# alinjar1996/manipulator_mujoco

Measured on AMD Instinct MI355X. Metric: candidate rollouts/sec (N×H steps) UR5e scene, 1/2/4/8 MI355X, higher is better.
Workload: dtype f32; 1 GPU; C3 scene_mjx: UR5e+Hand-E arm + object.xml box (URD/scene_mjx.xml), Newton(1 it, 5 ls), 4096 candidates x 50 steps per GPU, order-10 Bernstein, dt 0.05; candidates_per_gpu=4096, horizon=50, global_batch=4096, parallelism=dp1 (candidate shards; key exchange), world_size_seen=1, backend=single process, gpus_visible=1, launcher=single process, exchange=none (one rank: the fused atomic-min key is the global best)

## Files before the change

manipulator_mujoco_amd/build.py:

```python

from __future__ import annotations

import os
import shutil
import subprocess
import sys

HERE = os.path.dirname(os.path.abspath(__file__))
CSRC = os.path.join(HERE, "csrc")
_ROLLOUT_FLAGS = ["-Xarch_device", "-fno-slp-vectorize", "-Xarch_device", "-fassociative-math",
                  "-Xarch_device", "-fno-signed-zeros", "-Xarch_device", "-fno-trapping-math"]
UNITS = [(os.path.join(CSRC, "engine.hip"), [], False),
         (os.path.join(CSRC, "rollout_narrow.hip"), _ROLLOUT_FLAGS, False),
         (os.path.join(CSRC, "rollout_wide.hip"), _ROLLOUT_FLAGS, True)]
SRC = [u[0] for u in UNITS]
DEPS = SRC + [os.path.join(CSRC, f) for f in ("rollout.hip", "rollout.h", "cem.hip", "comm.hip",
                                              "mpcr_device.h", "mjcf_embed.cpp")] + [
    os.path.join(os.path.dirname(HERE), "include", f) for f in ("mpcr.h", "mpcr_model.h", "mpcr_mjcf.h")]
OUT = os.path.join(HERE, "libmpcr.so")
ARCH = os.environ.get("MPCR_OFFLOAD_ARCH", "gfx950")
FLAGS = ["-O3", "-std=c++17", "-fPIC", "-Wall", "-Wno-pass-failed",
         "-fno-hip-fp32-correctly-rounded-divide-sqrt", "-Xarch_device", "-freciprocal-math",
         "-Xarch_device", "-fapprox-func", "-mllvm", "-simplifycfg-sink-common=false"]


def source_hash() -> str:
    import hashlib
    h = hashlib.sha256()
    for d in DEPS:
        h.update(os.path.basename(d).encode())
        with open(d, "rb") as f:
            h.update(f.read())
    h.update(repr((FLAGS, [u[1:] for u in UNITS])).encode())
    return h.hexdigest()[:16]


def hipcc():
    for c in (os.environ.get("HIPCC"), "/opt/rocm/bin/hipcc", shutil.which("hipcc")):
        if c and os.path.exists(c):
            return c
    raise RuntimeError("hipcc not found")


FAST_MATH = {"-freciprocal-math", "-fapprox-func", "-fassociative-math", "-fno-signed-zeros", "-fno-trapping-math"}


def _drop_fast(flags):
    out, skip = [], False
    for i, f in enumerate(flags):
# ... 65 lines not shown
```

manipulator_mujoco_amd/csrc/engine.hip:

```cpp
#include <hip/hip_runtime.h>
#include <dlfcn.h>

#include <algorithm>
#include <atomic>
#include <cfloat>
#include <cmath>
#include <cstdarg>
#include <cstdio>
#include <cstring>
#include <limits>
#include <string>
#include <thread>
#include <vector>

#include "../../include/mpcr.h"
#include "mpcr_device.h"

#include "rollout.h"

#ifndef MPCR_SEG_STEPS_DEFAULT
#define MPCR_SEG_STEPS_DEFAULT 7
#endif
#ifndef MPCR_SEG_GROUPS_DEFAULT
#define MPCR_SEG_GROUPS_DEFAULT 2
#endif
#define MPCR_SEG_MAXG 4
static int env_int_or(const char* name, int dflt) {
  const char* v = getenv(name);
  return v ? atoi(v) : dflt;
}
#include "cem.hip"

namespace mpcr {
__global__ void __launch_bounds__(256) argmin_kernel(const float* __restrict__ cost, int stride, int n, int base,
                                                     unsigned long long* key) {
  unsigned long long best = ~0ull;
  for (int i = blockIdx.x * blockDim.x + threadIdx.x; i < n; i += gridDim.x * blockDim.x) {
    const float c = cost[(size_t)i * stride];
    const uint32_t u = __float_as_uint(c);
    const uint32_t k = isnan(c) ? 0u : ((u & 0x80000000u) ? ~u : (u | 0x80000000u));
    const unsigned long long k64 = ((unsigned long long)k << 32) | (uint32_t)(base + i);
    best = k64 < best ? k64 : best;
  }
#pragma unroll
  for (int o = 32; o > 0; o >>= 1) {
    const unsigned long long other = __shfl_xor(best, o);
    best = other < best ? other : best;
  }
  if ((threadIdx.x & 63) == 0) atomicMin(key, best);
}

// ... 14 lines not shown
  DevModel* d_model = nullptr;
  float* d_pdot = nullptr;
  float* d_in = nullptr;
  float* d_cost = nullptr;
  float* d_theta = nullptr;
  float* d_thetadot = nullptr;
  unsigned long long* d_key = nullptr;
  int* d_status = nullptr;
  int* d_idx = nullptr;
  float* d_slot_prev = nullptr;
  float* d_jx = nullptr;
  float* d_td = nullptr;
  short* d_hints = nullptr;
  unsigned* d_pace = nullptr;
  float* d_mslab = nullptr;
  float* d_seg = nullptr;
  int seg_steps = 0, seg_groups = 1, seg_min_n = 0;
  hipStream_t seg_stream[MPCR_SEG_MAXG] = {};
  hipEvent_t seg_event[MPCR_SEG_MAXG + 1] = {};
  float4* d_hull_vert = nullptr;
  int2* d_hull_info = nullptr;
  float4* d_hull_adjv = nullptr;
  float4* d_hull_head = nullptr;
  float4* d_hull_lut = nullptr;
  float4* d_face_plane = nullptr;
  int2* d_face_vinfo = nullptr;
  int* d_face_vert = nullptr;
  int2* d_vert_finfo = nullptr;
  int* d_vert_face = nullptr;
  int2* d_cone_cell = nullptr;
  int* d_cone_face = nullptr;
  bool wide = false;
};

static bool needs_wide(const mpcr_model_t& m, const DevModel& d) {
  if (m.nv > 16 || d.nbody > 16 || d.ngeom > 24 || m.nq > MPCR_N_NQ || m.nu > 0 || d.has_spring ||
      m.integrator != MPCR_INT_EULER || m.cone != MPCR_CONE_PYRAMIDAL || m.nten > 0 || m.viscosity != 0)
    return true;
  for (int e = 0; e < m.neq; e++)
    if (m.eq_type[e] != MPCR_EQ_JOINT) return true;
  for (int p = 0; p < m.npair; p++)
    if (m.pair_func[p] == MPCR_COL_CONVEX || m.pair_func[p] == MPCR_COL_PLANE_CONVEX) return true;
  return false;
}

static thread_local std::string g_err;

static int fail(int code, const char* fmt, ...) __attribute__((format(printf, 2, 3)));
static int fail(int code, const char* fmt, ...) {
  char buf[512];
  va_list ap;
  va_start(ap, fmt);
  vsnprintf(buf, sizeof(buf), fmt, ap);
  va_end(ap);
  g_err = buf;
  return code;
}

#define HIPCHK(x)                                                                         \
  do {                                                                                    \
    hipError_t e_ = (x);                                                                  \
    if (e_ != hipSuccess) return fail(MPCR_EHIP, "%s: %s", #x, hipGetErrorString(e_));  \
  } while (0)

extern "C" const char* mpcr_last_error(void) { return g_err.c_str(); }
extern "C" int mpcr_abi_version(void) { return MPCR_ABI_VERSION; }
// ... 847 lines not shown
        double ctr[3], cr[3];
        dir(0.5 * (u0 + u1), 0.5 * (v0 + v1), ctr);
        double rad = 0.0;
        for (double u : {u0, u1})
          for (double v : {v0, v1}) {
            dir(u, v, cr);
            const double cd = ctr[0] * cr[0] + ctr[1] * cr[1] + ctr[2] * cr[2];
            rad = std::max(rad, std::acos(std::min(1.0, cd)));
          }
        const double cth = std::cos(thr0 + rad);
        const int start = (int)cface.size();
        for (int f = fa; f < fa + fnum; f++) {
          const double* fp = h.face_plane[f];
          const double fn = std::sqrt(fp[0] * fp[0] + fp[1] * fp[1] + fp[2] * fp[2]);
          if (fn > 0 && (fp[0] * ctr[0] + fp[1] * ctr[1] + fp[2] * ctr[2]) / fn >= cth) cface.push_back(f);
        }
        ccell.push_back(make_int2(start, (int)cface.size() - start));
      }
    }
    if (cface.empty()) cface.push_back(0);
    if (ccell.empty()) ccell.push_back(make_int2(0, 0));
    if (hipMalloc(&e->d_cone_cell, sizeof(int2) * ccell.size()) != hipSuccess ||
        hipMalloc(&e->d_cone_face, sizeof(int) * cface.size()) != hipSuccess ||
        hipMemcpy(e->d_cone_cell, ccell.data(), sizeof(int2) * ccell.size(), hipMemcpyHostToDevice) != hipSuccess ||
        hipMemcpy(e->d_cone_face, cface.data(), sizeof(int) * cface.size(), hipMemcpyHostToDevice) != hipSuccess) {
      mpcr_engine_free(e);
      return fail(MPCR_ENOMEM, "cone table upload failed");
    }
    e->dev.cone_cell = as_gmem(e->d_cone_cell);
    e->dev.cone_face = as_gmem(e->d_cone_face);
  }
  const int nc = e->host.nctrl;
  const size_t in_cols = (size_t)nc * (horizon > nbasis ? horizon : nbasis);
  if (hipMalloc(&e->d_model, sizeof(DevModel)) != hipSuccess ||
      hipMalloc(&e->d_pdot, sizeof(float) * horizon * nbasis) != hipSuccess ||
      hipMalloc(&e->d_in, sizeof(float) * max_n * in_cols) != hipSuccess ||
      hipMalloc(&e->d_cost, sizeof(float) * max_n * 4) != hipSuccess ||
      hipMalloc(&e->d_theta, sizeof(float) * max_n * nc * horizon) != hipSuccess ||
      hipMalloc(&e->d_thetadot, sizeof(float) * max_n * nc * horizon) != hipSuccess ||
      hipMalloc(&e->d_key, sizeof(unsigned long long)) != hipSuccess ||
      hipMalloc(&e->d_status, sizeof(int) * max_n) != hipSuccess ||
      hipMalloc(&e->d_idx, sizeof(int) * max_n) != hipSuccess ||
      hipMalloc(&e->d_slot_prev, sizeof(float) * ((size_t)max_n + 1) * (e->host.nslot > 0 ? e->host.nslot : 1)) !=
          hipSuccess ||
      hipMalloc(&e->d_jx, sizeof(float) * ((size_t)max_n + 1) *
                              (e->wide ? (SmemW::MAXEFC - SmemW::JL + 1) * SmemW::LDJ
                                       : (SmemN::MAXEFC - SmemN::JL + 1) * SmemN::LDJ)) !=
          hipSuccess ||
      hipMalloc(&e->d_hints, sizeof(short) * 2 * (size_t)max_n * (e->wide ? SmemW::NHINT : 1)) != hipSuccess ||
      hipMalloc(&e->d_pace, sizeof(unsigned) * MPCR_PACE_SLOTS) != hipSuccess ||
      hipMalloc(&e->d_mslab, sizeof(float) * ((size_t)max_n + 1) * (e->wide ? SmemW::NVW * SmemW::LD : 1)) !=
          hipSuccess ||
      hipMalloc(&e->d_td, sizeof(float) * ((size_t)max_n + 1) * (size_t)(e->host.nctrl > 0 ? e->host.nctrl : 1) *
                              (size_t)horizon) != hipSuccess) {
    mpcr_engine_free(e);
    return fail(MPCR_ENOMEM, "device allocation failed");
  }
  if (hipMemcpy(e->d_model, &e->dev, sizeof(DevModel), hipMemcpyHostToDevice) != hipSuccess ||
      hipMemcpy(e->d_pdot, pdot, sizeof(float) * horizon * nbasis, hipMemcpyHostToDevice) != hipSuccess ||
      hipMemset(e->d_hints, 0xff, sizeof(short) * 2 * (size_t)max_n * (e->wide ? SmemW::NHINT : 1)) !=
          hipSuccess ||
      hipMemset(e->d_pace, 0xff, sizeof(unsigned) * MPCR_PACE_SLOTS) != hipSuccess) {
    mpcr_engine_free(e);
    return fail(MPCR_EHIP, "model upload failed");
  }
  if (e->wide) {
    e->seg_steps = env_int_or("MPCR_SEG_STEPS", MPCR_SEG_STEPS_DEFAULT);
    e->seg_groups = std::max(1, std::min(MPCR_SEG_MAXG, env_int_or("MPCR_SEG_GROUPS", MPCR_SEG_GROUPS_DEFAULT)));
    if (e->seg_steps > 0 && e->seg_steps < horizon) {
      int occ[6] = {0, 0, 0, 0, 0, 0}, ncu = 0;
      if (rollout_occupancy(occ) == hipSuccess &&
          hipDeviceGetAttribute(&ncu, hipDeviceAttributeMultiprocessorCount, device) == hipSuccess)
        e->seg_min_n = occ[3] * ncu;
      bool ok = hipMalloc(&e->d_seg, sizeof(float) * (size_t)max_n * SEG_STRIDE) == hipSuccess;
      for (int g = 0; ok && e->seg_groups > 1 && g < e->seg_groups; g++)
        ok = hipStreamCreateWithFlags(&e->seg_stream[g], hipStreamNonBlocking) == hipSuccess;
      for (int g = 0; ok && e->seg_groups > 1 && g <= e->seg_groups; g++)
        ok = hipEventCreateWithFlags(&e->seg_event[g], hipEventDisableTiming) == hipSuccess;
      if (!ok) {
        mpcr_engine_free(e);
        return fail(MPCR_ENOMEM, "horizon-segment state allocation failed");
      }
    }
  }
  *out = e;
  return MPCR_OK;
}

extern "C" void mpcr_engine_free(mpcr_engine* e) {
// ... 798 lines not shown
```

manipulator_mujoco_amd/csrc/rollout.hip:

```cpp
#pragma once
#include "rollout.h"
#include "../../include/mpcr_model.h"

namespace mpcr {

#ifdef MPCR_PROFILE
#define PROF_DECL unsigned long long prof_acc[32] = {0}; unsigned long long prof_last = __builtin_amdgcn_s_memtime();
#define STAMP(i)                                              \
  do {                                                        \
    unsigned long long now_ = __builtin_amdgcn_s_memtime();   \
    prof_acc[i] += now_ - prof_last;                          \
    prof_last = now_;                                         \
  } while (0)
#define PROF_FLUSH                                                          \
  if (lane == 0 && args.prof)                                               \
    for (int i_ = 0; i_ < 32; i_++) atomicAdd(&args.prof[i_ + 32 * (threadIdx.x >> 6)], prof_acc[i_]);
#ifdef MPCR_PROFILE_COUNTS
#define PROF_COUNT(m, i)                                                                  \
  do {                                                                                    \
    if ((m)->prof && (int)__lane_id() == __builtin_ctzll(__ballot(1))) atomicAdd((m)->prof + (i), 1ull); \
  } while (0)
#else
#define PROF_COUNT(m, i)
#endif
#define PSTAMP_DECL unsigned long long pst_ = __builtin_amdgcn_s_memtime();
#define PSTAMP(m, i)                                                                       \
  do {                                                                                     \
    const unsigned long long now_ = __builtin_amdgcn_s_memtime();                          \
    if ((m)->prof && (int)__lane_id() == 0) atomicAdd((m)->prof + (i) + 32 * (threadIdx.x >> 6), now_ - pst_); \
    pst_ = now_;                                                                           \
  } while (0)
#else
#define PSTAMP_DECL
#define PSTAMP(m, i)
// ... 8 lines not shown
  if (ahead >= 3) __builtin_amdgcn_s_setprio(3); \
  else if (ahead == 2) __builtin_amdgcn_s_setprio(2); \
  else if (ahead == 1) __builtin_amdgcn_s_setprio(1); \
  else __builtin_amdgcn_s_setprio(0); \
  }

#ifndef MPCR_CB_SKIP
#define MPCR_CB_SKIP 1
#endif
#ifdef MPCR_STOP_AFTER
#define STOP_AT(k) \
  if (MPCR_STOP_AFTER == (k)) continue;
#else
#define STOP_AT(k)
#endif


#if defined(__HIP_DEVICE_COMPILE__)
#define ASSUME_GLOBAL(p) __builtin_assume(!__builtin_amdgcn_is_shared((const void*)(p)) && \
                                          !__builtin_amdgcn_is_private((const void*)(p)))
#define ASSUME_LDS(p) __builtin_assume(__builtin_amdgcn_is_shared((const void*)(p)))
#define ASSUME_PRIVATE(p) __builtin_assume(__builtin_amdgcn_is_private((const void*)(p)))
#else
#define ASSUME_GLOBAL(p)
#define ASSUME_LDS(p)
#define ASSUME_PRIVATE(p)
#endif
__device__ __forceinline__ const MPCR_GMEM DevModel* uniform_model(const DevModel* p) {
  const unsigned long long a = reinterpret_cast<unsigned long long>(p);
  const unsigned lo = __builtin_amdgcn_readfirstlane((unsigned)a), hi = __builtin_amdgcn_readfirstlane((unsigned)(a >> 32));
  return reinterpret_cast<const MPCR_GMEM DevModel*>(((unsigned long long)hi << 32) | lo);
}

__device__ __forceinline__ float rdlane(float v, int l) {
  return __int_as_float(__builtin_amdgcn_readlane(__float_as_int(v), l));
}
template <int CTRL>
__device__ __forceinline__ float dppf(float v) {
  return __int_as_float(__builtin_amdgcn_update_dpp(0, __float_as_int(v), CTRL, 0xF, 0xF, false));
}
template <int CTRL, int ROWS>
__device__ __forceinline__ float dppf_rows(float v) {
  return __int_as_float(__builtin_amdgcn_update_dpp(0, __float_as_int(v), CTRL, ROWS, 0xF, false));
}
__device__ __forceinline__ float wsum(float v) {
  v += dppf<0xB1>(v);
  v += dppf<0x4E>(v);
  v += dppf<0x124>(v);
  v += dppf<0x128>(v);
  v += dppf_rows<0x142, 0xA>(v);
  v += dppf_rows<0x143, 0xC>(v);
  return rdlane(v, 63);
}
__device__ __forceinline__ int lanes_below(unsigned long long mask) {
  return (int)__builtin_amdgcn_mbcnt_hi((unsigned)(mask >> 32), __builtin_amdgcn_mbcnt_lo((unsigned)mask, 0u));
}
template <int BITS = 3>
__device__ __forceinline__ int wscan_excl(int v, int& total) {
  int pre = 0, tot = 0;
#pragma unroll
  for (int bit = 0; bit < BITS; bit++) {
    const unsigned long long mk = __ballot((v >> bit) & 1);
    pre += lanes_below(mk) << bit;
    tot += __popcll(mk) << bit;
  }
  total = tot;
// ... 2339 lines not shown
  float vnext = lane < nc ? tdp[lane * H + t_begin] : 0.f;
  float cost_g = 0.f, cost_r = 0.f, cost_c = 0.f;
  SlotHist<S> shist;
#pragma unroll
  for (int j = 0; j < SlotHist<S>::NC; j++)
#pragma unroll
    for (int c = 0; c < 4; c++) shist.v[j][c] = 0.f;
  int status = 0, nefc_sum = 0, nefc_max = 0;
  if (resume) {
    cost_c = segs[SEG_COSTC + lane];
    const float* sc = segs + SEG_SCAL;
    cost_g = sc[0]; cost_r = sc[1];
    status = __float_as_int(sc[2]); nefc_sum = __float_as_int(sc[3]); nefc_max = __float_as_int(sc[4]);
  }
  const int ctrl_qa = lane < nc ? m->ctrl_qposadr[lane] : 0, ctrl_da = lane < nc ? m->ctrl_dofadr[lane] : 0;
  PROF_DECL
  unsigned* pace = nullptr;
  int pace_own = 0;
  unsigned pace_v = ~0u;
  if (WPC == 1 && args.pace) {
    const unsigned hw = __builtin_amdgcn_s_getreg((31 << 11) | 4);
    const unsigned xcc = __builtin_amdgcn_s_getreg((3 << 11) | 20);
    const unsigned grp = ((((xcc & 7u) * 8u + ((hw >> 13) & 7u)) * 2u + ((hw >> 12) & 1u)) * 16u + ((hw >> 8) & 15u)) *
                             4u + ((hw >> 4) & 3u);
    pace = args.pace + grp * 16u;
    pace_own = (int)(hw & 15u);
  }
#ifdef MPCR_WAVETIME
  const unsigned long long wt_t0 = __builtin_amdgcn_s_memrealtime(), wt_c0 = __builtin_amdgcn_s_memtime();
  unsigned wt_newton = 0, wt_ls = 0, wt_cvx = 0;
#endif

  auto cdof_phase = [&]() {
    if (lane < nv) {
      const int bd = m->dof_body[lane], kind = m->dof_kind[lane];
      const int tr = m->body_tree[bd];
      float* c = s.cdof[lane];
      float R[9];
#pragma unroll
      for (int k = 0; k < 9; k++) R[k] = s.xmat[bd][k];
      if (kind == 2) {
        c[0] = c[1] = c[2] = 0.f;
        const int k = m->dof_sub[lane];
        c[3] = k == 0 ? 1.f : 0.f;
        c[4] = k == 1 ? 1.f : 0.f;
        c[5] = k == 2 ? 1.f : 0.f;
      } else {
        float ax[3], anchor[3];
        if (kind == 3) {
          const int k = m->dof_sub[lane];
          ax[0] = s.xmat[bd][k]; ax[1] = s.xmat[bd][3 + k]; ax[2] = s.xmat[bd][6 + k];
          anchor[0] = s.xpos[bd][0]; anchor[1] = s.xpos[bd][1]; anchor[2] = s.xpos[bd][2];
        } else {
          const int j = m->dof_jnt[lane];
          float w[3];
          mv(ax, R, m->jnt_axis[j]);
          mv(w, R, m->jnt_pos[j]);
          anchor[0] = s.xpos[bd][0] + w[0]; anchor[1] = s.xpos[bd][1] + w[1]; anchor[2] = s.xpos[bd][2] + w[2];
        }
        if (kind == 1) {
          c[0] = c[1] = c[2] = 0.f;
          c[3] = ax[0]; c[4] = ax[1]; c[5] = ax[2];
        } else {
          float off[3] = {s.com[tr][0] - anchor[0], s.com[tr][1] - anchor[1], s.com[tr][2] - anchor[2]}, cr[3];
          cross(cr, ax, off);
          c[0] = ax[0]; c[1] = ax[1]; c[2] = ax[2];
          c[3] = cr[0]; c[4] = cr[1]; c[5] = cr[2];
        }
      }
    }
  };
  for (int t = t_begin; t < t_end; t++) {
    LAUNDER_MODEL();
    LAUNDER_LANE();
    if (pace) {
      if (lane == pace_own) __hip_atomic_store(pace + lane, (unsigned)t, __ATOMIC_RELAXED, __HIP_MEMORY_SCOPE_WORKGROUP);
      if (lane < 16) pace_v = __hip_atomic_load(pace + lane, __ATOMIC_RELAXED, __HIP_MEMORY_SCOPE_AGENT);
    }
    if (run_main) {
    if (lane < nc) {
      const float v = vnext;
      if (t + 1 < H) vnext = tdp[lane * H + t + 1];
      s.qvel[ctrl_da] = v;
      if (args.layout != 0 && args.thetadot) args.thetadot[(size_t)b * nc * H + lane * H + t] = v;
    }
    sync();

    STAMP(0);
    STOP_AT(0)
    {
      float q[4] = {1.f, 0.f, 0.f, 0.f}, p[3] = {0.f, 0.f, 0.f};
      int anc = -1;
      if (lane < nb) {
        const int kind = m->body_kind[lane];
        const int j = m->body_jnt[lane];
        q[0] = m->body_bquat[lane][0]; q[1] = m->body_bquat[lane][1];
        q[2] = m->body_bquat[lane][2]; q[3] = m->body_bquat[lane][3];
        p[0] = m->body_bpos[lane][0]; p[1] = m->body_bpos[lane][1]; p[2] = m->body_bpos[lane][2];
        anc = m->body_anc[lane];
        if (kind == BK_FREE) {
          const int a = m->jnt_qposadr[j];
          p[0] = s.qpos[a]; p[1] = s.qpos[a + 1]; p[2] = s.qpos[a + 2];
          q[0] = s.qpos[a + 3]; q[1] = s.qpos[a + 4]; q[2] = s.qpos[a + 5]; q[3] = s.qpos[a + 6];
          float n = sqrtf(q[0] * q[0] + q[1] * q[1] + q[2] * q[2] + q[3] * q[3]);
          if (n < kMinVal) { q[0] = 1.f; q[1] = q[2] = q[3] = 0.f; }
          else { q[0] /= n; q[1] /= n; q[2] /= n; q[3] /= n; }
          anc = -1;
        } else if (kind == BK_HINGE || kind == BK_SLIDE) {
          const float qa = s.qpos[m->jnt_qposadr[j]] - m->jnt_qpos0[j];
          const float* ax = m->jnt_axis[j];
          float R[9];
          q2m(R, q);
          if (kind == BK_SLIDE) {
            float w[3];
            mv(w, R, ax);
            p[0] += w[0] * qa; p[1] += w[1] * qa; p[2] += w[2] * qa;
          } else {
            float sn, cs;
            __sincosf(0.5f * qa, &sn, &cs);
            float qj[4] = {cs, ax[0] * sn, ax[1] * sn, ax[2] * sn}, Rj[9], c[3], rc[3], d[3], w[3];
            c[0] = m->jnt_pos[j][0]; c[1] = m->jnt_pos[j][1]; c[2] = m->jnt_pos[j][2];
            q2m(Rj, qj);
            mv(rc, Rj, c);
            d[0] = c[0] - rc[0]; d[1] = c[1] - rc[1]; d[2] = c[2] - rc[2];
            mv(w, R, d);
            p[0] += w[0]; p[1] += w[1]; p[2] += w[2];
            qmul(q, q, qj);
          }
        }
      }
      for (int r = 0; r < m->jump_rounds; r++) {
        const int src = anc >= 0 ? anc : lane;
        float aq[4], ap[3];
        aq[0] = wshfl(q[0], src); aq[1] = wshfl(q[1], src);
        aq[2] = wshfl(q[2], src); aq[3] = wshfl(q[3], src);
        ap[0] = wshfl(p[0], src); ap[1] = wshfl(p[1], src); ap[2] = wshfl(p[2], src);
        const int aanc = wshfl(anc, src);
        if (anc >= 0) {
          float R[9], w[3];
          q2m(R, aq);
          mv(w, R, p);
          p[0] = ap[0] + w[0]; p[1] = ap[1] + w[1]; p[2] = ap[2] + w[2];
          qmul(q, aq, q);
          anc = aanc;
        }
      }
      if (lane < nb) {
        float n = sqrtf(q[0] * q[0] + q[1] * q[1] + q[2] * q[2] + q[3] * q[3]);
        q[0] /= n; q[1] /= n; q[2] /= n; q[3] /= n;
        float R[9], w[3];
        q2m(R, q);
        s.xpos[lane][0] = p[0]; s.xpos[lane][1] = p[1]; s.xpos[lane][2] = p[2];
        s.xquat[lane][0] = q[0]; s.xquat[lane][1] = q[1]; s.xquat[lane][2] = q[2]; s.xquat[lane][3] = q[3];
#pragma unroll
        for (int k = 0; k < 9; k++) s.xmat[lane][k] = R[k];
        mv(w, R, m->body_ipos[lane]);
        s.xipos[lane][0] = p[0] + w[0]; s.xipos[lane][1] = p[1] + w[1]; s.xipos[lane][2] = p[2] + w[2];
      }
    }
    sync();

    STAMP(1);
    STOP_AT(1)
    if (lane < m->ngeom) {
      const int gb = m->geom_body[lane];
      float gq[4] = {m->geom_quat[lane][0], m->geom_quat[lane][1], m->geom_quat[lane][2], m->geom_quat[lane][3]};
      float Rg[9];
      q2m(Rg, gq);
      if (gb < 0) {
        s.gxpos[lane][0] = m->geom_pos[lane][0]; s.gxpos[lane][1] = m->geom_pos[lane][1];
        s.gxpos[lane][2] = m->geom_pos[lane][2];
#pragma unroll
        for (int k = 0; k < 9; k++) s.gxmat[lane][k] = Rg[k];
      } else {
        float w[3], R[9], Rr[9];
#pragma unroll
        for (int k = 0; k < 9; k++) R[k] = s.xmat[gb][k];
        mv(w, R, m->geom_pos[lane]);
        s.gxpos[lane][0] = s.xpos[gb][0] + w[0]; s.gxpos[lane][1] = s.xpos[gb][1] + w[1];
        s.gxpos[lane][2] = s.xpos[gb][2] + w[2];
#pragma unroll
        for (int i = 0; i < 3; i++)
#pragma unroll
          for (int k = 0; k < 3; k++)
            Rr[3 * i + k] = R[3 * i] * Rg[k] + R[3 * i + 1] * Rg[3 + k] + R[3 * i + 2] * Rg[6 + k];
#pragma unroll
        for (int k = 0; k < 9; k++) s.gxmat[lane][k] = Rr[k];
      }
    }
// ... 618 lines not shown
        STAMP(18);
      }
      if (split && !lead && run_coll && lane == 0) s.ncon = ncon_w;
      sync();
      if (run_coll && s.ncon > S::MAXACT) {
        status |= 1;
        sync();
        if (lane == 0) s.ncon = S::MAXACT;
        sync();
      }
    }
    const bool rows_c = WPC == 2 && m->coll_rows;
    const bool rows_j = WPC == 2 && S::WIDE && !rows_c;
    const bool hess2 = rows_j && NVW == 32;
    const bool impl2 = hess2 && S::WIDE && m->integrator == 3 && !m->impl_cross && blk_usable<NVW>(m);
    constexpr int BLK_N = NVW == 16 ? 8 : 16;
    static_assert(!S::SPLIT || (BLK_N + 1) * WAVE <= S::DYN_FLOATS, "the implicit factor inside the dynamics region");
    float* const implf = &s.xpos[0][0];
    const int rl0 = rows_j ? wv * WAVE : 0, rls = rows_j ? 2 * WAVE : WAVE;
    if constexpr (WPC == 2) {
      if (!rows_c) {
        block_sync();
        if (!run_main && !rows_j) continue;
      }
    }

    STAMP(7);
    STOP_AT(7)
    bool coupled = true;
    if (WPC == 1 || rows_j || (rows_c ? run_coll : run_main)) {
      const int ncon = s.ncon;
      const int neq = (m->disableflags & 64) ? 0 : (S::WIDE ? m->neqrow : m->neq);
      int nlim_l = 0, lsides = 0;
      if (lane < m->njnt && !(m->disableflags & 32) && m->jnt_limited[lane] &&
          (m->jnt_type[lane] == 2 || m->jnt_type[lane] == 3)) {
        const float q = s.qpos[m->jnt_qposadr[lane]];
        if (q - m->jnt_range[lane][0] < m->jnt_margin[lane]) { nlim_l++; lsides |= 1; }
        if (m->jnt_range[lane][1] - q < m->jnt_margin[lane]) { nlim_l++; lsides |= 2; }
      }
      int nlim;
      const int lim_pre = wscan_excl(nlim_l, nlim);
      int ntr = 0, tsides = 0;
      if constexpr (S::WIDE) {
        if (!(m->disableflags & 32))
          for (int t = 0; t < m->nten; t++) {
            if (!m->ten_limited[t]) continue;
            const float dx = s.tenp[t][1][0] - s.tenp[t][0][0], dy = s.tenp[t][1][1] - s.tenp[t][0][1],
                        dz = s.tenp[t][1][2] - s.tenp[t][0][2];
            const float len = sqrtf(dx * dx + dy * dy + dz * dz);
            if (len - m->ten_range[t][0] < m->ten_margin[t]) { tsides |= 1 << (2 * t); ntr++; }
            if (m->ten_range[t][1] - len < m->ten_margin[t]) { tsides |= 2 << (2 * t); ntr++; }
          }
      }
      const bool ell = S::WIDE && m->cone == 1;
      int ncr = 0;
      if (lane < ncon) ncr = m->pair_condim[s.con_pair[lane]] == 1 ? 1 : (ell ? 3 : 4);
      int ncrow;
      const int con_pre = wscan_excl(ncr, ncrow);
      int nefc = neq + nlim + ntr + ncrow;
      int keep_con = ncon;
      if (nefc > S::MAXEFC) {
        const int room = S::MAXEFC - neq - nlim - ntr;
        const unsigned long long fit = __ballot(lane < ncon && con_pre + ncr <= room);
        keep_con = __popcll(fit);
        nefc = neq + nlim + ntr + (keep_con > 0 ? wshfl(con_pre + ncr, keep_con - 1) : 0);
        status |= 1;
// ... 103 lines not shown
                            s.con_pos[c][2] - s.com[tr][2]}, cr[3];
              cross(cr, cd, r);
              const float sg = side == 0 ? -1.f : 1.f;
              jd[0] += sg * (cd[3] + cr[0]); jd[1] += sg * (cd[4] + cr[1]); jd[2] += sg * (cd[5] + cr[2]);
            }
          }
        }
        float fw[9];
        const float* f = s.con_frame[c];
        if constexpr (S::FRAMEW == 3) {
          make_frame(fw, s.con_frame[c]);
          f = fw;
        }
        const float jn = f[0] * jd[0] + f[1] * jd[1] + f[2] * jd[2];
        const int off = s.con_row[c];
        if (m->pair_condim[p] == 1) {
          jstore(s, gx, off, i, jn);
        } else if (S::WIDE && m->cone == 1) {
          jstore(s, gx, off + 0, i, jn);
          jstore(s, gx, off + 1, i, f[3] * jd[0] + f[4] * jd[1] + f[5] * jd[2]);
          jstore(s, gx, off + 2, i, f[6] * jd[0] + f[7] * jd[1] + f[8] * jd[2]);
        } else {
          const float mu = m->pair_friction[p];
          const float jt1 = f[3] * jd[0] + f[4] * jd[1] + f[5] * jd[2];
          const float jt2 = f[6] * jd[0] + f[7] * jd[1] + f[8] * jd[2];
          jstore(s, gx, off + 0, i, jn + mu * jt1);
          jstore(s, gx, off + 1, i, jn - mu * jt1);
          jstore(s, gx, off + 2, i, jn + mu * jt2);
          jstore(s, gx, off + 3, i, jn - mu * jt2);
        }
      }
      if (rows_j) block_sync();
      else sync();
      for (int r = lane + rl0; r < nefc; r += rls) {
        const int src = s.efc_src[r], kind = src >> 24, id = (src >> 4) & 0xfffff, side = src & 15;
        float pos, margin, diag;
        const float* sref;
        const float* simp;
        if (S::WIDE && kind == 1 && side > 0) {
          pos = s.eqp[id][0][side - 1] - s.eqp[id][1][side - 1];
          margin = 0.f;
          diag = m->eq_diag[id];
          sref = m->eq_solref[id];
          simp = m->eq_solimp[id];
        } else if (kind == 1) {
          const int j1 = m->eq_j1[id], j2 = m->eq_j2[id];
          const float* c = m->eq_data[id];
          const float q1 = s.qpos[m->jnt_qposadr[j1]] - m->jnt_qpos0[j1];
          if (j2 >= 0) {
            const float dif = s.qpos[m->jnt_qposadr[j2]] - m->jnt_qpos0[j2];
            pos = q1 - (c[0] + dif * (c[1] + dif * (c[2] + dif * (c[3] + dif * c[4]))));
          } else {
            pos = q1 - c[0];
          }
          margin = 0.f;
          diag = m->eq_diag[id];
          sref = m->eq_solref[id];
          simp = m->eq_solimp[id];
        } else if (kind == 2) {
          const float q = s.qpos[m->jnt_qposadr[id]];
          pos = side == 0 ? q - m->jnt_range[id][0] : m->jnt_range[id][1] - q;
          margin = m->jnt_margin[id];
          diag = m->dof_invweight0[m->jnt_dofadr[id]];
          sref = m->jnt_solref[id];
          simp = m->jnt_solimp[id];
        } else if (S::WIDE && kind == 4) {
// ... 538 lines not shown
```

Baseline: 2.555 million rollouts/s.

## Add precomputed per-body/dof/row step table with packed float4 loads for narrow rollout

Builds a host-side step table of per-body kinematics constants, per-dof descriptors and per-constraint-row impedance and solref parameters (K, B, reciprocals, power flags). The table is packed as aligned float4 records and placed behind the device model. The narrow rollout kernel reads it in kinematics, cdof and constraint-row phases instead of scattered DevModel fields and per-step solimp/solref arithmetic. Intent is fewer scalar global loads and less repeated parameter math per step. The cost is extra device memory and a second code path that must stay consistent with the model, which a host-side equivalence check enforces.

```diff
diff --git a/manipulator_mujoco_amd/build.py b/manipulator_mujoco_amd/build.py
--- a/manipulator_mujoco_amd/build.py
+++ b/manipulator_mujoco_amd/build.py
@@ -14,7 +14,7 @@
          (os.path.join(CSRC, "rollout_narrow.hip"), _ROLLOUT_FLAGS, False),
          (os.path.join(CSRC, "rollout_wide.hip"), _ROLLOUT_FLAGS, True)]
 SRC = [u[0] for u in UNITS]
-DEPS = SRC + [os.path.join(CSRC, f) for f in ("rollout.hip", "rollout.h", "cem.hip", "comm.hip",
+DEPS = SRC + [os.path.join(CSRC, f) for f in ("rollout.hip", "rollout.h", "step_table.h", "cem.hip", "comm.hip",
                                               "mpcr_device.h", "mjcf_embed.cpp")] + [
     os.path.join(os.path.dirname(HERE), "include", f) for f in ("mpcr.h", "mpcr_model.h", "mpcr_mjcf.h")]
 OUT = os.path.join(HERE, "libmpcr.so")
diff --git a/manipulator_mujoco_amd/csrc/engine.hip b/manipulator_mujoco_amd/csrc/engine.hip
--- a/manipulator_mujoco_amd/csrc/engine.hip
+++ b/manipulator_mujoco_amd/csrc/engine.hip
@@ -17,6 +17,7 @@
 #include "mpcr_device.h"
 
 #include "rollout.h"
+#include "step_table.h"
 
 #ifndef MPCR_SEG_STEPS_DEFAULT
 #define MPCR_SEG_STEPS_DEFAULT 7
@@ -97,6 +98,47 @@
   int* d_cone_face = nullptr;
   bool wide = false;
 };
+
+static_assert(ST_NB == DX_NB && ST_NV == DX_NV && ST_NP == DX_NP && ST_NJ == DX_NJ && ST_NEQ == DX_NEQ,
+              "step table capacities = device model capacities");
+static_assert(ST_BK_FREE == BK_FREE && ST_BK_HINGE == BK_HINGE && ST_BK_SLIDE == BK_SLIDE && ST_BK_WELD == BK_WELD,
+              "body kinds");
+static_assert(ST_MINVAL == kMinVal && ST_MINIMP == kMinImp && ST_MAXIMP == kMaxImp, "the kernel's impedance constants");
+static bool step_table_matches(const StepTable& t, const DevModel& d) {
+  auto same = [](const float* a, const float* b, int n) { return std::memcmp(a, b, sizeof(float) * n) == 0; };
+  if (t.nbody != d.nbody) return false;
+  for (int i = 0; i < d.nbody; i++) {
+    const StepBody& r = t.body[i];
+    const int j = d.body_jnt[i];
+    if (r.kind != d.body_kind[i] || r.anc != d.body_anc[i] || r.qposadr != (j >= 0 ? d.jnt_qposadr[j] : -1)) return false;
+    if (!same(r.bquat, d.body_bquat[i], 4) || !same(r.bpos, d.body_bpos[i], 3) || !same(r.ipos, d.body_ipos[i], 3))
+      return false;
+    if (j >= 0 && r.qpos0 != d.jnt_qpos0[j]) return false;
+    if (r.kind == BK_HINGE && (!same(r.axis, d.jnt_axis[j], 3) || !same(r.jpos, d.jnt_pos[j], 3))) return false;
+  }
+  for (int i = 0; i < d.nv; i++) {
+    const StepDof& r = t.dof[i];
+    const int j = d.dof_jnt[i];
+    if (r.body != d.dof_body[i] || r.kind != d.dof_kind[i] || r.sub != d.dof_sub[i] ||
+        r.tree != (r.body >= 0 ? d.body_tree[r.body] : -1))
+      return false;
+    if (!same(r.axis, d.jnt_axis[j], 3) || !same(r.jpos, d.jnt_pos[j], 3)) return false;
+  }
+  for (int p = 0; p < d.npair; p++) {
+    const StepRow& r = t.row[ST_ROW_PAIR + p];
+    if (r.margin != d.pair_margin[p] || ((r.flags & ST_CONDIM1) != 0) != (d.pair_condim[p] == 1)) return false;
+  }
+  for (int j = 0; j < d.njnt; j++) {
+    const StepRow& r = t.row[ST_ROW_JNT + j];
+    const bool lim = d.jnt_limited[j] && (d.jnt_type[j] == MPCR_JNT_SLIDE || d.jnt_type[j] == MPCR_JNT_HINGE);
+    if (r.qposadr != d.jnt_qposadr[j] || r.dofadr != d.jnt_dofadr[j] || ((r.flags & ST_LIMITED) != 0) != lim ||
+        r.margin != d.jnt_margin[j] || r.diag != d.dof_invweight0[d.jnt_dofadr[j]] || !same(r.range, d.jnt_range[j], 2))
+      return false;
+  }
+  for (int q = 0; q < d.neq; q++)
+    if (t.row[ST_ROW_EQ + q].diag != d.eq_diag[q]) return false;
+  return true;
+}
 
 static bool needs_wide(const mpcr_model_t& m, const DevModel& d) {
   if (m.nv > 16 || d.nbody > 16 || d.ngeom > 24 || m.nq > MPCR_N_NQ || m.nu > 0 || d.has_spring ||
@@ -1010,7 +1052,8 @@
   }
   const int nc = e->host.nctrl;
   const size_t in_cols = (size_t)nc * (horizon > nbasis ? horizon : nbasis);
-  if (hipMalloc(&e->d_model, sizeof(DevModel)) != hipSuccess ||
+  static_assert(sizeof(DevModel) % alignof(mpcr::StepTable) == 0, "the step table's alignment behind the device model");
+  if (hipMalloc(reinterpret_cast<void**>(&e->d_model), sizeof(DevModel) + sizeof(StepTable)) != hipSuccess ||
       hipMalloc(&e->d_pdot, sizeof(float) * horizon * nbasis) != hipSuccess ||
       hipMalloc(&e->d_in, sizeof(float) * max_n * in_cols) != hipSuccess ||
       hipMalloc(&e->d_cost, sizeof(float) * max_n * 4) != hipSuccess ||
@@ -1033,6 +1076,21 @@
                               (size_t)horizon) != hipSuccess) {
     mpcr_engine_free(e);
     return fail(MPCR_ENOMEM, "device allocation failed");
+  }
+  if (!e->wide) {
+    std::vector<StepTable> step(1);
+    if (build_step_table(e->host, step[0]) != 0) {
+      mpcr_engine_free(e);
+      return fail(MPCR_EMODEL, "model exceeds the step table's capacities");
+    }
+    if (!step_table_matches(step[0], e->dev)) {
+      mpcr_engine_free(e);
+      return fail(MPCR_EMODEL, "step table and device model disagree (step_table.h / build_dev_model)");
+    }
+    if (hipMemcpy(e->d_model + 1, step.data(), sizeof(StepTable), hipMemcpyHostToDevice) != hipSuccess) {
+      mpcr_engine_free(e);
+      return fail(MPCR_EHIP, "step table upload failed");
+    }
   }
   if (hipMemcpy(e->d_model, &e->dev, sizeof(DevModel), hipMemcpyHostToDevice) != hipSuccess ||
       hipMemcpy(e->d_pdot, pdot, sizeof(float) * horizon * nbasis, hipMemcpyHostToDevice) != hipSuccess ||
diff --git a/manipulator_mujoco_amd/csrc/rollout.hip b/manipulator_mujoco_amd/csrc/rollout.hip
--- a/manipulator_mujoco_amd/csrc/rollout.hip
+++ b/manipulator_mujoco_amd/csrc/rollout.hip
@@ -1,5 +1,6 @@
 #pragma once
 #include "rollout.h"
+#include "step_table.h"
 #include "../../include/mpcr_model.h"
 
 namespace mpcr {
@@ -74,6 +75,20 @@
   return reinterpret_cast<const MPCR_GMEM DevModel*>(((unsigned long long)hi << 32) | lo);
 }
 
+#ifndef MPCR_STEP_TABLE
+#define MPCR_STEP_TABLE 7
+#endif
+template <class S> constexpr bool kStepKin = !S::WIDE && (MPCR_STEP_TABLE & 1) != 0;
+template <class S> constexpr bool kStepDof = !S::WIDE && (MPCR_STEP_TABLE & 2) != 0;
+template <class S> constexpr bool kStepRow = !S::WIDE && (MPCR_STEP_TABLE & 4) != 0;
+__device__ __forceinline__ const StepTable* step_table(const DevModel* m) {
+  return reinterpret_cast<const StepTable*>(m + 1);
+}
+template <class R>
+__device__ __forceinline__ float4 recq(const R& r, int q) {
+  return reinterpret_cast<const float4*>(&r)[q];
+}
+
 __device__ __forceinline__ float rdlane(float v, int l) {
   return __int_as_float(__builtin_amdgcn_readlane(__float_as_int(v), l));
 }
@@ -2479,6 +2494,49 @@
 #endif
 
   auto cdof_phase = [&]() {
+    if constexpr (kStepDof<S>) {
+      if (lane < nv) {
+        const StepTable* st = step_table(m);
+        const float4 d0 = recq(st->dof[lane], 0);
+        const int bd = __float_as_int(d0.x), kind = __float_as_int(d0.y), tr = __float_as_int(d0.z),
+                  k = __float_as_int(d0.w);
+        float* c = s.cdof[lane];
+        if (kind == 2) {
+          c[0] = c[1] = c[2] = 0.f;
+          c[3] = k == 0 ? 1.f : 0.f;
+          c[4] = k == 1 ? 1.f : 0.f;
+          c[5] = k == 2 ? 1.f : 0.f;
+        } else {
+          float ax[3], anchor[3] = {s.xpos[bd][0], s.xpos[bd][1], s.xpos[bd][2]};
+          if (kind == 3) {
+            ax[0] = s.xmat[bd][k]; ax[1] = s.xmat[bd][3 + k]; ax[2] = s.xmat[bd][6 + k];
+          } else {
+            const float4 d1 = recq(st->dof[lane], 1);
+            const float ja[3] = {d1.x, d1.y, d1.z};
+            float R[9];
+#pragma unroll
+            for (int i = 0; i < 9; i++) R[i] = s.xmat[bd][i];
+            mv(ax, R, ja);
+            if (!(st->flags & ST_ANCHOR0)) {
+              const float4 d2 = recq(st->dof[lane], 2);
+              const float jp[3] = {d2.x, d2.y, d2.z};
+              float w[3];
+              mv(w, R, jp);
+              anchor[0] += w[0]; anchor[1] += w[1]; anchor[2] += w[2];
+            }
+          }
+          if (kind == 1) {
+            c[0] = c[1] = c[2] = 0.f;
+            c[3] = ax[0]; c[4] = ax[1]; c[5] = ax[2];
+          } else {
+            float off[3] = {s.com[tr][0] - anchor[0], s.com[tr][1] - anchor[1], s.com[tr][2] - anchor[2]}, cr[3];
+            cross(cr, ax, off);
+            c[0] = ax[0]; c[1] = ax[1]; c[2] = ax[2];
+            c[3] = cr[0]; c[4] = cr[1]; c[5] = cr[2];
+          }
+        }
+      }
+    } else {
     if (lane < nv) {
       const int bd = m->dof_body[lane], kind = m->dof_kind[lane];
       const int tr = m->body_tree[bd];
@@ -2516,6 +2574,7 @@
         }
       }
     }
+    }
   };
   for (int t = t_begin; t < t_end; t++) {
     LAUNDER_MODEL();
@@ -2538,6 +2597,46 @@
     {
       float q[4] = {1.f, 0.f, 0.f, 0.f}, p[3] = {0.f, 0.f, 0.f};
       int anc = -1;
+      if constexpr (kStepKin<S>) {
+        if (lane < nb) {
+          const StepTable* st = step_table(m);
+          const float4 b0 = recq(st->body[lane], 0), b1 = recq(st->body[lane], 1), b2 = recq(st->body[lane], 2);
+          const int kind = __float_as_int(b0.x), qa0 = __float_as_int(b0.z);
+          anc = __float_as_int(b0.y);
+          q[0] = b1.x; q[1] = b1.y; q[2] = b1.z; q[3] = b1.w;
+          p[0] = b2.x; p[1] = b2.y; p[2] = b2.z;
+          if (kind == BK_FREE) {
+            const int a = qa0;
+            p[0] = s.qpos[a]; p[1] = s.qpos[a + 1]; p[2] = s.qpos[a + 2];
+            q[0] = s.qpos[a + 3]; q[1] = s.qpos[a + 4]; q[2] = s.qpos[a + 5]; q[3] = s.qpos[a + 6];
+            float n = sqrtf(q[0] * q[0] + q[1] * q[1] + q[2] * q[2] + q[3] * q[3]);
+            if (n < kMinVal) { q[0] = 1.f; q[1] = q[2] = q[3] = 0.f; }
+            else { q[0] /= n; q[1] /= n; q[2] /= n; q[3] /= n; }
+          } else if (kind == BK_HINGE || kind == BK_SLIDE) {
+            const float qa = s.qpos[qa0] - b0.w;
+            const float4 b3 = recq(st->body[lane], 3);
+            if (kind == BK_SLIDE) {
+              p[0] += b3.x * qa; p[1] += b3.y * qa; p[2] += b3.z * qa;
+            } else {
+              float sn, cs;
+              __sincosf(0.5f * qa, &sn, &cs);
+              float qj[4] = {cs, b3.x * sn, b3.y * sn, b3.z * sn};
+              if (!(st->flags & ST_ANCHOR0)) {
+                const float4 b5 = recq(st->body[lane], 5), r0 = recq(st->body[lane], 6), r1 = recq(st->body[lane], 7),
+                             r2 = recq(st->body[lane], 8);
+                const float R[9] = {r0.x, r0.y, r0.z, r1.x, r1.y, r1.z, r2.x, r2.y, r2.z};
+                float Rj[9], c[3] = {b5.x, b5.y, b5.z}, rc[3], d[3], w[3];
+                q2m(Rj, qj);
+                mv(rc, Rj, c);
+                d[0] = c[0] - rc[0]; d[1] = c[1] - rc[1]; d[2] = c[2] - rc[2];
+                mv(w, R, d);
+                p[0] += w[0]; p[1] += w[1]; p[2] += w[2];
+              }
+              qmul(q, q, qj);
+            }
+          }
+        }
+      } else {
       if (lane < nb) {
         const int kind = m->body_kind[lane];
         const int j = m->body_jnt[lane];
@@ -2576,6 +2675,7 @@
           }
         }
       }
+      }
       for (int r = 0; r < m->jump_rounds; r++) {
         const int src = anc >= 0 ? anc : lane;
         float aq[4], ap[3];
@@ -2601,7 +2701,13 @@
         s.xquat[lane][0] = q[0]; s.xquat[lane][1] = q[1]; s.xquat[lane][2] = q[2]; s.xquat[lane][3] = q[3];
 #pragma unroll
         for (int k = 0; k < 9; k++) s.xmat[lane][k] = R[k];
-        mv(w, R, m->body_ipos[lane]);
+        if constexpr (kStepKin<S>) {
+          const float4 b4 = recq(step_table(m)->body[lane], 4);
+          const float ip[3] = {b4.x, b4.y, b4.z};
+          mv(w, R, ip);
+        } else {
+          mv(w, R, m->body_ipos[lane]);
+        }
         s.xipos[lane][0] = p[0] + w[0]; s.xipos[lane][1] = p[1] + w[1]; s.xipos[lane][2] = p[2] + w[2];
       }
     }
@@ -3286,6 +3392,17 @@
       const int ncon = s.ncon;
       const int neq = (m->disableflags & 64) ? 0 : (S::WIDE ? m->neqrow : m->neq);
       int nlim_l = 0, lsides = 0;
+      if constexpr (kStepRow<S>) {
+        if (lane < m->njnt && !(m->disableflags & 32)) {
+          const StepRow& rj = step_table(m)->row[ST_ROW_JNT + lane];
+          const float4 j2 = recq(rj, 2), j3 = recq(rj, 3);
+          if (__float_as_int(j2.z) & ST_LIMITED) {
+            const float q = s.qpos[__float_as_int(j3.z)];
+            if (q - j3.x < j2.x) { nlim_l++; lsides |= 1; }
+            if (j3.y - q < j2.x) { nlim_l++; lsides |= 2; }
+          }
+        }
+      } else
       if (lane < m->njnt && !(m->disableflags & 32) && m->jnt_limited[lane] &&
           (m->jnt_type[lane] == 2 || m->jnt_type[lane] == 3)) {
         const float q = s.qpos[m->jnt_qposadr[lane]];
@@ -3455,6 +3572,60 @@
       }
       if (rows_j) block_sync();
       else sync();
+      if constexpr (kStepRow<S>) {
+        for (int r = lane + rl0; r < nefc; r += rls) {
+          const int src = s.efc_src[r], kind = src >> 24, id = (src >> 4) & 0xfffff, side = src & 15;
+          const StepTable* st = step_table(m);
+          float pos;
+          int ri;
+          if (kind == 1) {
+            const int j1 = m->eq_j1[id], j2 = m->eq_j2[id];
+            const float* c = m->eq_data[id];
+            const float q1 = s.qpos[m->jnt_qposadr[j1]] - m->jnt_qpos0[j1];
+            if (j2 >= 0) {
+              const float dif = s.qpos[m->jnt_qposadr[j2]] - m->jnt_qpos0[j2];
+              pos = q1 - (c[0] + dif * (c[1] + dif * (c[2] + dif * (c[3] + dif * c[4]))));
+            } else {
+              pos = q1 - c[0];
+            }
+            ri = ST_ROW_EQ + id;
+          } else if (kind == 2) {
+            ri = ST_ROW_JNT + id;
+            const float4 j3 = recq(st->row[ri], 3);
+            const float q = s.qpos[__float_as_int(j3.z)];
+            pos = side == 0 ? q - j3.x : j3.y - q;
+          } else {
+            ri = ST_ROW_PAIR + s.con_pair[id];
+            pos = s.con_dist[id];
+          }
+          const float4 a0 = recq(st->row[ri], 0), a1 = recq(st->row[ri], 1), a2 = recq(st->row[ri], 2);
+          const float vel = jdot(s, gx, r, s.qvel);
+          const float dpos = pos - a2.x;
+          const float x = fabsf(dpos * a0.z);
+          float imp;
+          if (x >= 1.f) {
+            imp = a0.y;
+          } else if (x <= 0.f) {
+            imp = a0.x;
+          } else {
+            const int fl = __float_as_int(a2.z);
+            const float mid = a0.w, power = a2.w;
+            float y;
+            if (fl & ST_POW1) y = x;
+            else if (fl & ST_POW2) y = x <= mid ? x * x * a1.x : 1.f - (1.f - x) * (1.f - x) * a1.y;
+            else if (x <= mid) y = powf(x, power) / powf(mid, power - 1.f);
+            else y = 1.f - powf(1.f - x, power) / powf(1.f - mid, power - 1.f);
+            imp = a0.x + y * (a0.y - a0.x);
+          }
+          const float R = fmaxf((1.f - imp) / imp * a2.y, kMinVal);
+          s.efc_D[r] = 1.f / R;
+          s.efc_aref[r] = -a1.w * vel - a1.z * imp * dpos;
+          if (args.dbg && b == 0 && t == H - 1 && r < DBG_MAXROW) {
+            float* o = args.dbg + DBG_ROW + 3 * r;
+            o[0] = s.efc_D[r]; o[1] = s.efc_aref[r]; o[2] = vel;
+          }
+        }
+      } else
       for (int r = lane + rl0; r < nefc; r += rls) {
         const int src = s.efc_src[r], kind = src >> 24, id = (src >> 4) & 0xfffff, side = src & 15;
         float pos, margin, diag;
diff --git a/manipulator_mujoco_amd/csrc/step_table.h b/manipulator_mujoco_amd/csrc/step_table.h
--- /dev/null
+++ b/manipulator_mujoco_amd/csrc/step_table.h
@@ -0,0 +1,229 @@
+#pragma once
+#include <math.h>
+#include <stdint.h>
+#include <string.h>
+
+#include "../../include/mpcr_model.h"
+
+namespace mpcr {
+
+constexpr int ST_NB = 32, ST_NV = 32, ST_NP = 768, ST_NJ = 32, ST_NEQ = 8;
+constexpr int ST_ROW_PAIR = 0, ST_ROW_JNT = ST_NP, ST_ROW_EQ = ST_NP + ST_NJ, ST_NROW = ST_NP + ST_NJ + ST_NEQ;
+constexpr float ST_MINVAL = 1e-15f, ST_MINIMP = 0.0001f, ST_MAXIMP = 0.9999f;
+
+enum { ST_ANCHOR0 = 1 };
+enum {
+  ST_POW2 = 1,
+  ST_POW1 = 2,
+  ST_LIMITED = 4,
+  ST_CONDIM1 = 8
+};
+enum { ST_BK_FREE = 1, ST_BK_HINGE = 2, ST_BK_SLIDE = 3, ST_BK_WELD = 4 };
+
+struct alignas(16) StepBody {
+  int32_t kind, anc, qposadr;
+  float qpos0;
+  float bquat[4];
+  float bpos[3], pad0;
+  float axis[3], pad1;
+  float ipos[3], pad2;
+  float jpos[3], pad3;
+  float R[3][4];
+};
+struct alignas(16) StepDof {
+  int32_t body, kind, tree, sub;
+  float axis[3], pad0;
+  float jpos[3], pad1;
+};
+struct alignas(16) StepRow {
+  float dmin, dmax, iwidth, mid;
+  float imid, i1mid, K, B;
+  float margin, diag;
+  int32_t flags;
+  float power;
+  float range[2];
+  int32_t qposadr, dofadr;
+};
+
+struct alignas(16) StepTable {
+  int32_t flags, nbody, pad[2];
+  StepBody body[ST_NB];
+  StepDof dof[ST_NV];
+  StepRow row[ST_NROW];
+};
+
+namespace step_detail {
+inline void qmul(double r[4], const double a[4], const double b[4]) {
+  const double t[4] = {a[0] * b[0] - a[1] * b[1] - a[2] * b[2] - a[3] * b[3],
+                       a[0] * b[1] + a[1] * b[0] + a[2] * b[3] - a[3] * b[2],
+                       a[0] * b[2] - a[1] * b[3] + a[2] * b[0] + a[3] * b[1],
+                       a[0] * b[3] + a[1] * b[2] - a[2] * b[1] + a[3] * b[0]};
+  memcpy(r, t, sizeof(t));
+}
+inline void q2m(double m[9], const double q[4]) {
+  const double w = q[0], x = q[1], y = q[2], z = q[3];
+  m[0] = 1 - 2 * (y * y + z * z); m[1] = 2 * (x * y - w * z); m[2] = 2 * (x * z + w * y);
+  m[3] = 2 * (x * y + w * z); m[4] = 1 - 2 * (x * x + z * z); m[5] = 2 * (y * z - w * x);
+  m[6] = 2 * (x * z - w * y); m[7] = 2 * (y * z + w * x); m[8] = 1 - 2 * (x * x + y * y);
+}
+inline void rot(double r[3], const double q[4], const double v[3]) {
+  double m[9];
+  q2m(m, q);
+  for (int i = 0; i < 3; i++) r[i] = m[3 * i] * v[0] + m[3 * i + 1] * v[1] + m[3 * i + 2] * v[2];
+}
+inline double clampd(double x, double lo, double hi) { return x < lo ? lo : (x > hi ? hi : x); }
+
+inline void row_params(StepRow& r, const double solref[2], const double solimp[5], double timestep, int disableflags) {
+  double dmin = clampd(solimp[0], (double)ST_MINIMP, (double)ST_MAXIMP);
+  double dmax = clampd(solimp[1], (double)ST_MINIMP, (double)ST_MAXIMP);
+  double width = solimp[2], mid = solimp[3];
+  const double power = solimp[4];
+  const bool flat = (float)dmin == (float)dmax || (float)width <= ST_MINVAL;
+  double iwidth = 1.0 / width, imid = 1.0 / mid, i1mid = 1.0 / (1.0 - mid);
+  if (flat) {
+    dmin = dmax = 0.5 * ((double)(float)dmin + (double)(float)dmax);
+    iwidth = 0.0; mid = 0.5; imid = 2.0; i1mid = 2.0;
+  }
+  const double d = clampd(solimp[1], (double)ST_MINIMP, (double)ST_MAXIMP);
+  double tc = solref[0];
+  const double dr = solref[1];
+  double K, B;
+  if ((float)tc > 0.f) {
+    if (!(disableflags & MPCR_DSBL_REFSAFE) && tc < 2.0 * timestep) tc = 2.0 * timestep;
+    K = 1.0 / (d * d * tc * tc * dr * dr);
+    B = 2.0 / (d * tc);
+  } else {
+    K = -tc / (d * d);
+    B = -dr / d;
+  }
+  r.dmin = (float)dmin; r.dmax = (float)dmax; r.iwidth = (float)iwidth; r.mid = (float)mid;
+  r.imid = (float)imid; r.i1mid = (float)i1mid; r.K = (float)K; r.B = (float)B;
+  r.power = (float)power;
+  r.flags = flat ? ST_POW1 : ((float)power == 2.f ? ST_POW2 : ((float)power == 1.f ? ST_POW1 : 0));
+}
+}
+
+inline int build_step_table(const mpcr_model_t& m, StepTable& t) {
+  using namespace step_detail;
+  memset(&t, 0, sizeof(t));
+  if (m.nbody > MPCR_MAX_BODY || m.njnt > ST_NJ || m.nv > ST_NV || m.npair > ST_NP || m.neq > ST_NEQ)
+    return -1;
+  int dmap[MPCR_MAX_BODY], nb = 0;
+  double wpos[MPCR_MAX_BODY][3] = {}, wquat[MPCR_MAX_BODY][4] = {};
+  dmap[0] = -1;
+  wquat[0][0] = 1;
+  for (int b = 1; b < m.nbody; b++) dmap[b] = m.body_weldid[b] != 0 ? nb++ : -1;
+  if (nb > ST_NB) return -1;
+  for (int b = 1; b < m.nbody; b++) {
+    if (dmap[b] >= 0) continue;
+    const int p = m.body_parentid[b];
+    double r[3];
+    rot(r, wquat[p], m.body_pos[b]);
+    for (int k = 0; k < 3; k++) wpos[b][k] = wpos[p][k] + r[k];
+    qmul(wquat[b], wquat[p], m.body_quat[b]);
+    const double n = sqrt(wquat[b][0] * wquat[b][0] + wquat[b][1] * wquat[b][1] + wquat[b][2] * wquat[b][2] +
+                          wquat[b][3] * wquat[b][3]);
+    for (int k = 0; k < 4; k++) wquat[b][k] /= n;
+  }
+  int roots[MPCR_MAX_BODY], nroot = 0, btree[ST_NB];
+  for (int b = 1; b < m.nbody; b++) {
+    if (dmap[b] < 0) continue;
+    int tr = -1;
+    for (int k = 0; k < nroot; k++)
+      if (roots[k] == m.body_rootid[b]) tr = k;
+    if (tr < 0) { roots[nroot] = m.body_rootid[b]; tr = nroot++; }
+    btree[dmap[b]] = tr;
+  }
+  t.nbody = nb;
+  bool anchor0 = true;
+  for (int b = 1; b < m.nbody; b++) {
+    const int i = dmap[b];
+    if (i < 0) continue;
+    StepBody& r = t.body[i];
+    const int p = m.body_parentid[b];
+    const int j = m.body_jntnum[b] ? m.body_jntadr[b] : -1;
+    r.kind = j < 0 ? ST_BK_WELD
+                   : (m.jnt_type[j] == MPCR_JNT_FREE ? ST_BK_FREE
+                                                     : (m.jnt_type[j] == MPCR_JNT_HINGE ? ST_BK_HINGE : ST_BK_SLIDE));
+    double bq[4], bp[3];
+    if (dmap[p] < 0) {
+      double w[3];
+      rot(w, wquat[p], m.body_pos[b]);
+      for (int k = 0; k < 3; k++) bp[k] = wpos[p][k] + w[k];
+      qmul(bq, wquat[p], m.body_quat[b]);
+      r.anc = -1;
+    } else {
+      memcpy(bp, m.body_pos[b], sizeof(bp));
+      memcpy(bq, m.body_quat[b], sizeof(bq));
+      r.anc = dmap[p];
+    }
+    if (r.kind == ST_BK_FREE) r.anc = -1;
+    r.qposadr = j >= 0 ? m.jnt_qposadr[j] : -1;
+    r.qpos0 = j >= 0 ? (float)m.qpos0[m.jnt_qposadr[j]] : 0.f;
+    double R[9];
+    q2m(R, bq);
+    for (int k = 0; k < 4; k++) r.bquat[k] = (float)bq[k];
+    for (int k = 0; k < 3; k++) {
+      r.bpos[k] = (float)bp[k];
+      r.ipos[k] = (float)m.body_ipos[b][k];
+      for (int c = 0; c < 3; c++) r.R[k][c] = (float)R[3 * k + c];
+    }
+    if (r.kind == ST_BK_HINGE || r.kind == ST_BK_SLIDE) {
+      for (int k = 0; k < 3; k++) {
+        const double* a = m.jnt_axis[j];
+        r.axis[k] = r.kind == ST_BK_HINGE ? (float)a[k] : (float)(R[3 * k] * a[0] + R[3 * k + 1] * a[1] + R[3 * k + 2] * a[2]);
+        r.jpos[k] = (float)m.jnt_pos[j][k];
+        if (r.jpos[k] != 0.f) anchor0 = false;
+      }
+    }
+  }
+  t.flags = anchor0 ? ST_ANCHOR0 : 0;
+  for (int i = 0; i < m.nv; i++) {
+    StepDof& r = t.dof[i];
+    const int j = m.dof_jntid[i], sub = i - m.jnt_dofadr[j];
+    r.body = dmap[m.dof_bodyid[i]];
+    r.kind = m.jnt_type[j] == MPCR_JNT_HINGE ? 0 : (m.jnt_type[j] == MPCR_JNT_SLIDE ? 1 : (sub < 3 ? 2 : 3));
+    r.tree = r.body >= 0 ? btree[r.body] : -1;
+    r.sub = sub < 3 ? sub : sub - 3;
+    for (int k = 0; k < 3; k++) { r.axis[k] = (float)m.jnt_axis[j][k]; r.jpos[k] = (float)m.jnt_pos[j][k]; }
+  }
+  for (int p = 0; p < m.npair; p++) {
+    StepRow& r = t.row[ST_ROW_PAIR + p];
+    row_params(r, m.pair_solref[p], m.pair_solimp[p], m.timestep, m.disableflags);
+    const double mu = m.pair_friction[p];
+    const double invw = m.body_invweight0[m.geom_bodyid[m.pair_geom1[p]]][0] +
+                        m.body_invweight0[m.geom_bodyid[m.pair_geom2[p]]][0];
+    r.margin = (float)(m.pair_margin[p] - m.pair_gap[p]);
+    r.diag = (float)(m.pair_condim[p] == 1 ? invw : invw * (1.0 + mu * mu));
+    if (m.pair_condim[p] == 1) r.flags |= ST_CONDIM1;
+    r.qposadr = r.dofadr = -1;
+  }
+  for (int j = 0; j < m.njnt; j++) {
+    StepRow& r = t.row[ST_ROW_JNT + j];
+    row_params(r, m.jnt_solref[j], m.jnt_solimp[j], m.timestep, m.disableflags);
+    r.margin = (float)m.jnt_margin[j];
+    r.diag = (float)m.dof_invweight0[m.jnt_dofadr[j]];
+    if (m.jnt_limited[j] && (m.jnt_type[j] == MPCR_JNT_SLIDE || m.jnt_type[j] == MPCR_JNT_HINGE)) r.flags |= ST_LIMITED;
+    r.range[0] = (float)m.jnt_range[j][0];
+    r.range[1] = (float)m.jnt_range[j][1];
+    r.qposadr = m.jnt_qposadr[j];
+    r.dofadr = m.jnt_dofadr[j];
+  }
+  for (int e = 0; e < m.neq; e++) {
+    StepRow& r = t.row[ST_ROW_EQ + e];
+    row_params(r, m.eq_solref[e], m.eq_solimp[e], m.timestep, m.disableflags);
+    double diag = 0;
+    if (m.eq_type[e] == MPCR_EQ_JOINT) {
+      diag = m.dof_invweight0[m.jnt_dofadr[m.eq_obj1[e]]];
+      if (m.eq_obj2[e] >= 0) diag += m.dof_invweight0[m.jnt_dofadr[m.eq_obj2[e]]];
+    } else if (m.eq_type[e] == MPCR_EQ_CONNECT) {
+      diag = m.body_invweight0[m.eq_obj1[e]][0] + m.body_invweight0[m.eq_obj2[e]][0];
+    }
+    r.margin = 0.f;
+    r.diag = (float)diag;
+    r.qposadr = r.dofadr = -1;
+  }
+  return 0;
+}
+
+}
```

Measured after the change: 2.684 million rollouts/s (median of 6 runs). 1.05x the previous value.
